# Genie-Kim/PintheMemory

Hardware: AMD Instinct MI355X
Metric: train imgs/sec 768x768 bs=8 R50-DeepLabV3+ +mem (higher is better)
Workload: dtype f32

## Files before the change

include/pinmem_hip.h:

```cpp
#ifndef PINMEM_HIP_H
#define PINMEM_HIP_H
#include <stddef.h>
#include <stdint.h>

#ifdef __cplusplus
extern "C" {
#endif

typedef enum pm_status { PM_OK = 0, PM_EINVAL = -1, PM_EWORKSPACE = -2, PM_ELAUNCH = -3, PM_EUNSUPPORTED = -4 } pm_status;

typedef enum pm_dtype { PM_F32 = 0, PM_BF16 = 1 } pm_dtype;
#define PM_TF_ZERO_PAD64 1

typedef struct pm_tensor {
  void* ptr;
  int32_t n, h, w, c;
  int64_t pitch;
  int32_t dtype;
  int32_t flags;
} pm_tensor;

#define PM_ABI_VERSION 400

typedef struct pm_conv_params {
// ... 6 lines not shown
  int64_t wxf_bytes;
  int32_t wxf_valid;
} pm_conv_params;

typedef struct pm_conv_epilogue {
  int64_t struct_size;
  const float* bias;
  const float* scale;
  const float* shift;
  const float* residual;
  int64_t residual_pitch;
  int32_t relu;
  float* bn_partials;
  int64_t bn_partials_bytes;
} pm_conv_epilogue;

const char* pm_last_error(void);
int pm_version(void);

size_t pm_conv_workspace(const pm_tensor* x, const pm_tensor* y, const pm_conv_params* p, int which );
size_t pm_conv_winograd_v_bytes(const pm_tensor* x, const pm_tensor* y, const pm_conv_params* p);
size_t pm_conv_wxf_bytes(const pm_tensor* x, const pm_tensor* y, const pm_conv_params* p);
size_t pm_conv_wxf_bytes_dgrad(const pm_tensor* dy, const pm_tensor* dx, const pm_conv_params* p);
typedef struct pm_wxf_job {
  const float* w;
  void* wxf;
  int64_t wxf_bytes;
  int32_t cout, kh, kw, cin;
  int32_t dgrad;
  int32_t reserved;
} pm_wxf_job;
int pm_conv_wxf_refresh_bf16(const pm_wxf_job* jobs, int n, void* stream);
int pm_conv_wxf_refresh_f32(const pm_wxf_job* jobs, int n, void* stream);
size_t pm_conv_bn_partials_bytes(const pm_tensor* x, const pm_tensor* y, const pm_conv_params* p);
int pm_conv_fwd(const pm_tensor* x, const float* w_krsc, const pm_tensor* y, const pm_conv_params* p,
                const pm_conv_epilogue* ep, void* ws, size_t ws_bytes, void* stream);
int pm_conv_bwd_data(const pm_tensor* dy, const float* w_krsc, const pm_tensor* dx, const pm_conv_params* p,
                     const pm_tensor* add, void* ws, size_t ws_bytes, void* stream);
int pm_conv_bwd_data_masked(const pm_tensor* dy, const float* w_krsc, const pm_tensor* dx, const pm_conv_params* p,
                            const pm_tensor* add, const uint8_t* add_mask, void* ws, size_t ws_bytes, void* stream);
int pm_conv_bwd_weight(const pm_tensor* x, const pm_tensor* dy, float* dw_krsc, float* dbias, const pm_conv_params* p,
                       void* ws, size_t ws_bytes, void* stream);

typedef struct pm_routing {
  int32_t struct_size;
  int32_t winograd;
// ... 158 lines not shown
```

pinthememory_amd/csrc/conv_igemm.hip:

```cpp
#include <stdlib.h>
#include <algorithm>
#include <type_traits>
#include <vector>

#include "pm_common.h"

#include "conv_igemm_kernel.h"

namespace {

template <int ZL, bool O16 = false>
__global__ __launch_bounds__(256) void splitk_reduce_vec_kernel(const float* __restrict__ ws, int ksplit, long slab, int M, int Nn,
                                                                float* __restrict__ C, long c_pitch, const float* bias,
                                                                const float* scale, const float* shift, const float* residual,
                                                                long res_pitch, int relu, const unsigned char* res_mask) {
  constexpr int GP = 256 / ZL;
  __shared__ float4 red[ZL > 1 ? ZL : 1][GP];
  const int gl = threadIdx.x % GP, zl = threadIdx.x / GP;
  const long groups = (long)M * Nn / 4;
  for (long g0 = (long)blockIdx.x * GP; g0 < groups; g0 += (long)gridDim.x * GP) {
    const long grp = g0 + gl;
    float4 v = make_float4(0.f, 0.f, 0.f, 0.f);
    if (grp < groups)
#pragma unroll 8
// ... 841 lines not shown
  R_S2_PARITY,
  R_WINO_WGRAD,
  R_BF16_WGRAD,
  R_DIRECT_WGRAD,
};
struct ConvRoute {
  RouteKind kind;
  Plan pl;
  WinoPlan wino;
  WinoWgradPlan wino_w;
  Bf16Plan b16;
  pm_conv_params pe;
  S2Native s2n;
  S2ParityPlan s2p;
  Bf16WgradPlan b16w;
  W16Plan w16;
  bool native16;
  size_t ws_bytes;
  size_t class_off, slab_off;
  size_t bias_off;
  size_t x32_off, dy32_off;
  size_t v_keep_bytes;
  size_t wxf_bytes;
  size_t bn_bytes;
};

ConvRoute route_conv(int which, const pm_tensor* x, const pm_tensor* y, const pm_conv_params* p) {
  ConvRoute r{};
  long M, Nn, K;
  gemm_dims(which, x, y, p, M, Nn, K);
  if (which == MODE_FWD) {
    if ((r.wino = wino_plan(x, y->c, p)).use) {
      r.kind = R_WINO, r.ws_bytes = wino_ws(r.wino), r.wxf_bytes = r.wino.u_bytes;
      r.v_keep_bytes = wino_wgrad_pays(x->c, y->c) ? r.wino.v_bytes : 0;
    } else if (p->prec == 2 && (r.b16 = bf16_plan(x, y, p)).use) {
      r.kind = R_BF16, r.pe = *p, r.ws_bytes = bf16_ws(r.b16), r.wxf_bytes = r.b16.wb_bytes;
    } else {
      r.kind = R_DIRECT, r.pl = make_plan(MODE_FWD, M, Nn, K, p->prec != 0), r.ws_bytes = pm_align_up(r.pl.ws_bytes, 256);
    }
    bool bn;
    if (pm_is_bf16(y)) bn = pm_vec8(y) && r.kind == R_BF16 && (r.b16.c16 ? (r.b16.k16.ksplit == 1 && !r.b16.k16.wide) : r.b16.pl.ksplit == 1);
    else if (pm_is_bf16(x) || (y->c & 3) || (y->pitch & 3) || !pm_aligned16(y->ptr)) bn = false;
    else bn = r.kind == R_BF16 ? r.b16.pl.ksplit == 1 : (r.kind == R_DIRECT && p->prec == 0 && r.pl.ksplit == 1 && r.pl.bn >= 64);
    r.bn_bytes = bn ? pm_align_up((size_t)pm_cdiv(pm_pixels(y), 32) * y->c * 2 * sizeof(float), 256) : 0;
  } else if (which == MODE_DGRAD) {
    if (p->stride == 2) {
      if ((r.s2n = s2_native_plan(y, x, p)).ok) {
        r.kind = R_S2_NATIVE, r.ws_bytes = r.s2n.total;
      } else {
        r.kind = R_S2_PARITY, r.s2p = s2_parity_plan(y, x, p);
        r.class_off = 0, r.slab_off = 4 * r.s2p.tmp_bytes;
        r.dy32_off = pm_align_up(r.slab_off + r.s2p.slab_bytes + 256, 256);
        r.ws_bytes = r.dy32_off + upcast_bytes(y);
      }
    } else if (dgrad_bf16_ok(p) && (r.pe = dgrad_as_fwd(p), r.b16 = bf16_plan(y, x, &r.pe)).use) {
      r.kind = R_BF16, r.ws_bytes = bf16_ws(r.b16), r.wxf_bytes = r.b16.wb_bytes;
    } else if ((r.wino = wino_plan(y, x->c, p)).use) {
      r.kind = R_WINO, r.ws_bytes = wino_ws(r.wino);
    } else {
      r.kind = R_DIRECT, r.pl = make_plan(MODE_DGRAD, M, Nn, K, p->prec != 0), r.ws_bytes = pm_align_up(r.pl.ws_bytes, 256);
    }
  } else {
    const bool tier = pm_is_bf16(x) || pm_is_bf16(y);
    r.native16 = pm_is_bf16(x) && pm_is_bf16(y) && y->c >= 32;
    size_t own;
    if (!tier && (r.b16w = bf16_wgrad_plan(x, y, p)).use) {
      r.kind = R_BF16_WGRAD, own = bf16_wgrad_ws(r.b16w);
    } else if (!tier && (r.wino = wino_plan(x, y->c, p, true)).use) {
      r.kind = R_WINO_WGRAD, r.wino_w = wino_wgrad_plan(r.wino, y->c), own = wino_wgrad_ws(r.wino, r.wino_w);
    } else {
      r.kind = R_DIRECT_WGRAD, r.pl = make_plan(MODE_WGRAD, M, Nn, K, p->prec != 0), own = r.pl.ws_bytes;
      if (r.native16) {
        r.pl.kper = (r.pl.kper + 63) / 64 * 64;
        r.pl.ksplit = (int)((K + r.pl.kper - 1) / r.pl.kper);
        r.w16 = wgrad16_plan(x, y, p, M, Nn, K, r.pl.ksplit);
      }
    }
    r.bias_off = pm_align_up(own, 256);
    r.ws_bytes = r.bias_off + pm_align_up((size_t)pm_cdiv(pm_pixels(y), colsum_rows(pm_pixels(y), y->c)) * y->c * sizeof(float), 256) + upcast_bytes(x) + upcast_bytes(y);
    r.x32_off = r.dy32_off = r.ws_bytes;
    if (!r.native16) r.x32_off -= upcast_bytes(x);
// ... 203 lines not shown
  fclose(f);
  return PM_OK;
}

extern "C" size_t pm_conv_workspace(const pm_tensor* x, const pm_tensor* y, const pm_conv_params* p0, int which) {
  const pm_conv_params tp = tier_params(p0, x, y);
  return route_conv(which, x, y, &tp).ws_bytes;
}
extern "C" size_t pm_conv_winograd_v_bytes(const pm_tensor* x, const pm_tensor* y, const pm_conv_params* p0) {
  if (!x || !y || !p0) return 0;
  const pm_conv_params tp = tier_params(p0, x, y);
  return route_conv(MODE_FWD, x, y, &tp).v_keep_bytes;
}
extern "C" size_t pm_conv_wxf_bytes(const pm_tensor* x, const pm_tensor* y, const pm_conv_params* p0) {
  if (!x || !y || !p0) return 0;
  const pm_conv_params tp = tier_params(p0, x, y);
  return route_conv(MODE_FWD, x, y, &tp).wxf_bytes;
}
extern "C" size_t pm_conv_wxf_bytes_dgrad(const pm_tensor* dy, const pm_tensor* dx, const pm_conv_params* p0) {
  if (!dy || !dx || !p0) return 0;
  const pm_conv_params tp = tier_params(p0, dy, dx);
  return route_conv(MODE_DGRAD, dx, dy, &tp).wxf_bytes;
}
extern "C" size_t pm_conv_bn_partials_bytes(const pm_tensor* x, const pm_tensor* y, const pm_conv_params* p0) {
  if (!x || !y || !p0 || check_common(x, y, p0) != PM_OK) return 0;
  const pm_conv_params tp = tier_params(p0, x, y);
  return route_conv(MODE_FWD, x, y, &tp).bn_bytes;
}

extern "C" int pm_conv_wxf_refresh_f32(const pm_wxf_job* jobs, int n, void* stream) {
  PM_REQUIRE(n >= 0 && (jobs || n == 0), PM_EINVAL, "conv_wxf_refresh_f32: bad job table");
  std::vector<const float*> w(n);
  std::vector<float*> U(n);
  std::vector<int> cout(n), cin(n), kp(n), m(n);
  for (int i = 0; i < n; ++i) {
    const pm_wxf_job& q = jobs[i];
    PM_REQUIRE(q.w && q.wxf && q.cout > 0 && q.cin > 0 && q.kh == 3 && q.kw == 3 && q.dgrad == 0, PM_EINVAL,
               "conv_wxf_refresh_f32: job %d: forward transforms of 3x3 filters only", i);
    PM_REQUIRE(pm_aligned16(q.wxf), PM_EINVAL, "conv_wxf_refresh_f32: job %d: buffer must be 16-byte aligned", i);
    const int Kp = (q.cin + BK - 1) / BK * BK;
    const size_t u4 = pm_align_up((size_t)36 * q.cout * Kp * sizeof(float), 256), u2 = pm_align_up((size_t)16 * q.cout * Kp * sizeof(float), 256);
    PM_REQUIRE((size_t)q.wxf_bytes == u4 || (size_t)q.wxf_bytes == u2, PM_EINVAL, "conv_wxf_refresh_f32: job %d: %ld bytes is neither the F(4x4) nor the F(2x2) transform of %d x %d",
               i, (long)q.wxf_bytes, q.cout, q.cin);
    w[i] = q.w, U[i] = (float*)q.wxf, cout[i] = q.cout, cin[i] = q.cin, kp[i] = Kp, m[i] = (size_t)q.wxf_bytes == u4 ? 4 : 2;
  }
  return pm_wino_filter_xf_multi(w.data(), U.data(), cout.data(), cin.data(), kp.data(), m.data(), n, (hipStream_t)stream);
}

extern "C" int pm_conv_fwd(const pm_tensor* x, const float* w, const pm_tensor* y, const pm_conv_params* p0,
                           const pm_conv_epilogue* ep, void* ws, size_t ws_bytes, void* stream) {
  if (int e = check_common(x, y, p0)) return e;
  const pm_conv_params tp = tier_params(p0, x, y);
  const pm_conv_params* p = &tp;
  PM_REQUIRE(!ep || ep->struct_size == (int64_t)sizeof(pm_conv_epilogue), PM_EINVAL,
             "conv_fwd: pm_conv_epilogue.struct_size %ld != %zu -- caller built against another pinmem_hip.h (library ABI %d)", ep ? (long)ep->struct_size : 0l,
             sizeof(pm_conv_epilogue), PM_ABI_VERSION);
  PM_REQUIRE(w && pm_aligned16(w), PM_EINVAL, "conv_fwd: weight null or unaligned");
  pm_conv_epilogue e0 = {(int64_t)sizeof(pm_conv_epilogue), nullptr, nullptr, nullptr, nullptr, 0, 0};
  if (ep) e0 = *ep;
  PM_REQUIRE((e0.scale == nullptr) == (e0.shift == nullptr), PM_EINVAL, "conv_fwd: scale and shift go together");
  const ConvRoute r = route_conv(MODE_FWD, x, y, p);
  if (e0.bn_partials) {
    PM_REQUIRE(!e0.relu && !e0.residual, PM_EINVAL, "conv_fwd: bn_partials are the statistics of the convolution output (no residual / ReLU)");
    PM_REQUIRE(r.bn_bytes != 0 && (size_t)e0.bn_partials_bytes >= r.bn_bytes, PM_EINVAL, "conv_fwd: this call cannot emit bn_partials (ask pm_conv_bn_partials_bytes): %zu needed", r.bn_bytes);
  }
  PM_REQUIRE(ws_bytes >= r.ws_bytes && (ws || r.ws_bytes == 0), PM_EWORKSPACE, "conv_fwd: workspace %zu < %zu", ws_bytes, r.ws_bytes);
  hipStream_t st = (hipStream_t)stream;
  switch (r.kind) {
    case R_WINO: {
// ... 21 lines not shown
  if (int e = check_common(dx, dy, p0)) return e;
  const pm_conv_params tp = tier_params(p0, dy, dx);
  const pm_conv_params* p = &tp;
  PM_REQUIRE(!add || (add->ptr && pm_same_shape(add, dx) && add->dtype == dx->dtype), PM_EINVAL, "conv_bwd_data: `add` must match dx (shape and dtype)");
  PM_REQUIRE(!add || !pm_is_bf16(add) || pm_vec8(add), PM_EINVAL, "conv_bwd_data: bf16 `add` must be 16B aligned with pitch %% 8 == 0");
  PM_REQUIRE(w && pm_aligned16(w), PM_EINVAL, "conv_bwd_data: weight null or unaligned");
  const ConvRoute r = route_conv(MODE_DGRAD, dx, dy, p);
  PM_REQUIRE(ws_bytes >= r.ws_bytes && (ws || r.ws_bytes == 0), PM_EWORKSPACE, "conv_bwd_data: workspace %zu < %zu", ws_bytes, r.ws_bytes);
  if (add_mask) {
    PM_REQUIRE(add && pm_is_f32(add) && pm_is_f32(dy) && pm_vec4(add) && pm_vec4(dx), PM_EINVAL, "conv_bwd_data: a masked `add` is an fp32 tensor with 16-byte rows and c %% 4 == 0");
    PM_REQUIRE(r.kind == R_DIRECT, PM_EUNSUPPORTED,
               "conv_bwd_data: a masked `add` is served by the fp32 implicit-GEMM route only (this call routes to %s)",
               r.kind == R_WINO ? "Winograd" : (r.kind == R_BF16 ? "the bf16 kernels" : "the stride-2 class kernels"));
  }
  hipStream_t st = (hipStream_t)stream;
  const pm_conv_epilogue e1 = {(int64_t)sizeof(pm_conv_epilogue), nullptr, nullptr, nullptr, add ? (const float*)add->ptr : nullptr, add ? add->pitch : 0, 0};
  switch (r.kind) {
    case R_S2_NATIVE: return dgrad_s2_bf16(dy, w, dx, p, add, r.s2n, ws, st);
    case R_S2_PARITY: return dgrad_s2_parity(dy, w, dx, p, add, r, ws, st);
    case R_BF16: {
      char* wext = (p->wxf && (size_t)p->wxf_bytes >= r.b16.wb_bytes) ? (char*)p->wxf : nullptr;
      return conv_bf16(dy, w, dy->c, dx->c, true, dx, &r.pe, r.b16, e1, ws, st, wext, p->wxf_valid != 0);
    }
    case R_WINO: return wino_conv(dy, w, dy->c, dx->c, true, dx, r.wino, e1, ws, st);
    default:
      PM_REQUIRE(pm_is_f32(dy), PM_EUNSUPPORTED, "conv_bwd_data: a bf16 dy needs at least 32 channels and a stride-1 geometry the forward form covers");
      return conv_direct<MODE_DGRAD>(dx, dy, w, p, r.pl, e1, ws, st, add_mask);
  }
}

extern "C" int pm_conv_bwd_weight(const pm_tensor* x0, const pm_tensor* dy0, float* dw, float* dbias, const pm_conv_params* p0, void* ws,
                                  size_t ws_bytes, void* stream) {
  if (int e = check_common(x0, dy0, p0)) return e;
  const pm_conv_params tp = tier_params(p0, x0, dy0);
  const pm_conv_params* p = &tp;
  PM_REQUIRE(dw && pm_aligned16(dw), PM_EINVAL, "conv_bwd_weight: dw null or unaligned");
  const ConvRoute r = route_conv(MODE_WGRAD, x0, dy0, p);
  PM_REQUIRE(ws && ws_bytes >= r.ws_bytes, PM_EWORKSPACE, "conv_bwd_weight: workspace %zu < %zu", ws_bytes, r.ws_bytes);
  hipStream_t st = (hipStream_t)stream;
  const pm_tensor *x = x0, *dy = dy0;
  pm_tensor x32, dy32;
  if (!r.native16 && pm_is_bf16(x0)) {
    if (int e = upcast(x0, (char*)ws + r.x32_off, &x32, st)) return e;
    x = &x32;
  }
  if (pm_is_bf16(dy0) && (!r.native16 || dbias)) {
    if (int e = upcast(dy0, (char*)ws + r.dy32_off, &dy32, st)) return e;
// ... 21 lines not shown
```

pinthememory_amd/csrc/pm_common.h:

```cpp
#pragma once
#include <hip/hip_runtime.h>
#include <algorithm>
#include <atomic>
#include <stdarg.h>
#include <stdint.h>
#include <stdio.h>

#include "../../include/pinmem_hip.h"

void pm_set_error(const char* fmt, ...);

#define PM_REQUIRE(cond, code, ...)      \
  do {                                   \
    if (!(cond)) {                       \
      pm_set_error(__VA_ARGS__);         \
      return (code);                     \
    }                                    \
  } while (0)

static inline int pm_check_launch(const char* what) {
  hipError_t e = hipGetLastError();
  if (e != hipSuccess) {
    pm_set_error("%s: launch failed: %s", what, hipGetErrorString(e));
    return PM_ELAUNCH;
  }
  return PM_OK;
}

static inline bool pm_aligned16(const void* p) { return (reinterpret_cast<uintptr_t>(p) & 15u) == 0; }
static inline int64_t pm_pixels(const pm_tensor* t) { return (int64_t)t->n * t->h * t->w; }
static inline int pm_cdiv(int64_t a, int64_t b) { return (int)((a + b - 1) / b); }
static inline size_t pm_align_up(size_t v, size_t a) { return (v + a - 1) / a * a; }

static inline bool pm_vec_ok(const pm_tensor* t) { return pm_aligned16(t->ptr) && (t->pitch % 4) == 0; }
static inline bool pm_is_f32(const pm_tensor* t) { return t->dtype == PM_F32; }
static inline bool pm_is_bf16(const pm_tensor* t) { return t->dtype == PM_BF16; }
#define PM_REQUIRE_F32(t, who) PM_REQUIRE(!(t) || pm_is_f32(t), PM_EUNSUPPORTED, "%s: fp32 tensors only (got dtype %d)", who, (t)->dtype)
static inline bool pm_vec8(const pm_tensor* t) { return pm_is_bf16(t) && pm_aligned16(t->ptr) && (t->pitch % 8) == 0 && (t->c % 8) == 0; }

struct pm_wino_geom {
  int N, H, W, d, m, TY, TX;
  long tiles;
};
pm_wino_geom pm_wino_make_geom(int n, int h, int w, int d, int m);
int pm_wino_input_xf(const float* x, long pitch, int C, int Kp, const pm_wino_geom& g, float* V, hipStream_t st);
int pm_wino_filter_xf(const float* w, int Cout, int Cin, int Kp, bool dgrad, int m, float* U, hipStream_t st);
int pm_wino_filter_xf_multi(const float* const* w, float* const* U, const int* cout, const int* cin, const int* kp, const int* m, int n, hipStream_t st);
int pm_wino_output_xf(const float* M, int Cout, const pm_wino_geom& g, float* y, long ypitch, const float* bias, const float* scale, const float* shift,
                      const float* residual, long res_pitch, int relu, hipStream_t st);
int pm_wino_fused_f4(const float* V, const float* U, int Cout, int Kp, const pm_wino_geom& g, float* y, long ypitch, const float* bias, const float* scale,
                     const float* shift, const float* residual, long res_pitch, int relu, hipStream_t st);
int pm_wino_dy_xf(const float* dy, long pitch, int Cout, const pm_wino_geom& g, float* Z, hipStream_t st);
int pm_wino_dw_xf(const float* slab, int ks, int Cout, int Cin, int Kp, int m, float* dw, hipStream_t st);

int pm_bf16_cast_rows(const float* x, long pitch, int C, int Cp, long P, void* out, hipStream_t st);
int pm_bf16_cast_weights(const float* w, int Cout, int T, int Cin, int Cp, bool rotate, void* out, hipStream_t st);
struct PmS2Classes {
  int ky0[4], nky[4], kx0[4], nkx[4];
  void* out[4];
};
int pm_bf16_cast_weights_s2(const float* w, int Cout, int kh, int kw, int Cin, int Cp, const PmS2Classes* cl, hipStream_t st);
int pm_bf16_transpose_taps(const float* x, long pitch, int C, int N, int H, int W, int Ho, int Wo, int kh, int kw, int stride, int pad, int dil, void* out,
                           hipStream_t st);

typedef unsigned short pm_bf16;
int pm16_bn_stats(const pm_tensor* x, float* moments, float eps, float* mean, float* invstd, float* running_mean, float* running_var, float momentum, void* ws,
                  size_t ws_bytes, hipStream_t st);
size_t pm16_bn_workspace(const pm_tensor* x);
int pm16_bn_apply_mask(const pm_tensor* x, const float* mean, const float* invstd, const float* gamma, const float* beta, const pm_tensor* res, int relu,
                       const pm_tensor* y, uint8_t* mask, hipStream_t st);
// ... 183 lines not shown
      const long op = (long)(n * Ho + oy) * Wo + ox;
      const unsigned a = *reinterpret_cast<const unsigned*>(arg + op * C + ch), want = (unsigned)(ky * 3 + kx);
      const float4 d = *reinterpret_cast<const float4*>(dy + op * dp + ch);
      g.x += (a & 255u) == want ? d.x : 0.f;
      g.y += ((a >> 8) & 255u) == want ? d.y : 0.f;
      g.z += ((a >> 16) & 255u) == want ? d.z : 0.f;
      g.w += (a >> 24) == want ? d.w : 0.f;
    }
  }
  return g;
}

__device__ __forceinline__ float pm_wave_sum(float v) {
#pragma unroll
  for (int o = 32; o > 0; o >>= 1) v += __shfl_xor(v, o, 64);
  return v;
}
__device__ __forceinline__ float pm_wave_max(float v) {
#pragma unroll
  for (int o = 32; o > 0; o >>= 1) v = fmaxf(v, __shfl_xor(v, o, 64));
  return v;
}

struct pm_lerp {
  int i0, i1;
  float w0, w1;
};
__host__ __device__ __forceinline__ float pm_ac_scale(int in, int out) {
  return out > 1 ? (float)(in - 1) / (float)(out - 1) : 0.f;
}
__device__ __forceinline__ pm_lerp pm_ac_lerp(float scale, int dst, int in) {
  float src = scale * (float)dst;
  int i0 = (int)src;
  if (i0 > in - 1) i0 = in - 1;
  int i1 = i0 + (i0 < in - 1 ? 1 : 0);
  float l1 = src - (float)i0;
  if (l1 < 0.f) l1 = 0.f;
  if (l1 > 1.f) l1 = 1.f;
  pm_lerp r;
  r.i0 = i0;
  r.i1 = i1;
  r.w1 = l1;
  r.w0 = 1.f - l1;
  return r;
}

// ... 23 lines not shown
```

pinthememory_amd/csrc/winograd.hip:

```cpp
#include "pm_common.h"

namespace {

enum { W_BT = 0, W_AT = 1, W_G = 2, W_A = 3, W_GT = 4 };

template <int MT>
__host__ __device__ constexpr float wino_bt(int i, int j) {
  if (MT == 2) {
    constexpr float t[4][4] = {{1, 0, -1, 0}, {0, 1, 1, 0}, {0, -1, 1, 0}, {0, 1, 0, -1}};
    return t[i & 3][j & 3];
  }
  constexpr float t[6][6] = {{4, 0, -5, 0, 1, 0}, {0, -4, -4, 1, 1, 0}, {0, 4, -4, -1, 1, 0}, {0, -2, -1, 2, 1, 0}, {0, 2, -1, -2, 1, 0}, {0, 4, 0, -5, 0, 1}};
  return t[i][j];
}
template <int MT>
__host__ __device__ constexpr float wino_at(int i, int j) {
  if (MT == 2) {
    constexpr float t[2][4] = {{1, 1, 1, 0}, {0, 1, -1, -1}};
    return t[i & 1][j & 3];
  }
  constexpr float t[4][6] = {{1, 1, 1, 1, 1, 0}, {0, 1, -1, 2, -2, 0}, {0, 1, 1, 4, 4, 0}, {0, 1, -1, 8, -8, 1}};
  return t[i][j];
}
template <int MT>
// ... 68 lines not shown

struct TileId {
  int n, ry, rx, ty, tx;
};
__device__ __forceinline__ TileId decode_tile(unsigned tile, const pm_wino_geom& g) {
  TileId t;
  t.tx = (int)(tile % (unsigned)g.TX);
  unsigned q = tile / (unsigned)g.TX;
  t.ty = (int)(q % (unsigned)g.TY);
  q /= (unsigned)g.TY;
  t.rx = (int)(q % (unsigned)g.d);
  q /= (unsigned)g.d;
  t.ry = (int)(q % (unsigned)g.d);
  t.n = (int)(q / (unsigned)g.d);
  return t;
}

template <int MT, int W>
__global__ __launch_bounds__(256) void wino_input_kernel(const float* __restrict__ x, long xp, int C, int Kp, const pm_wino_geom g, float* __restrict__ V) {
  constexpr int A = MT + 2;
  const unsigned kg = Kp / W;
  const unsigned total = (unsigned)g.tiles * kg;
  const long plane = g.tiles * (long)Kp;
  for (unsigned i = blockIdx.x * 256u + threadIdx.x; i < total; i += gridDim.x * 256u) {
    const unsigned tile = i / kg;
    const int c = (int)(i - tile * kg) * W;
    const TileId t = decode_tile(tile, g);
    const bool cok = c < C;
    Vec<W> tt[A][A];
#pragma unroll
    for (int b = 0; b < A; ++b) {
      const int xx = t.rx + g.d * (MT * t.tx + b - 1);
      const bool xok = cok && (unsigned)xx < (unsigned)g.W;
      Vec<W> col[A], o[A];
#pragma unroll
      for (int a = 0; a < A; ++a) {
        const int yy = t.ry + g.d * (MT * t.ty + a - 1);
        col[a] = (xok && (unsigned)yy < (unsigned)g.H) ? vload<W>(x + ((long)(t.n * g.H + yy) * g.W + xx) * xp + c) : vzero<W>();
      }
      mat_apply<MT, W_BT>(col, o);
#pragma unroll
      for (int a = 0; a < A; ++a) tt[a][b] = o[a];
    }
    float* out = V + (long)tile * Kp + c;
#pragma unroll
    for (int a = 0; a < A; ++a) {
      Vec<W> o[A];
// ... 100 lines not shown
#pragma unroll
  for (int a = 0; a < A; ++a) {
    Vec<4> o[A];
    mat_apply<MT, W_G>(gg[a], o);
#pragma unroll
    for (int b = 0; b < A; ++b) {
#pragma unroll
      for (int e = 0; e < 4; ++e)
        if (k + e >= Kr) o[b].v[e] = 0.f;
      vstore<4>(out + (a * A + b) * plane, o[b]);
    }
  }
}
template <int MT, bool DGRAD>
__global__ __launch_bounds__(256) void wino_filter_kernel(const float* __restrict__ w, int Cout, int Cin, int Kp, float* __restrict__ U) {
  __shared__ float sg[9][32][33];
  wino_filter_block<MT, DGRAD>(w, Cout, Cin, Kp, U, blockIdx.x, blockIdx.y, sg);
}

constexpr int WR_BATCH = 48;
struct WinoRefreshJobs {
  const float* w[WR_BATCH];
  float* U[WR_BATCH];
  int cout[WR_BATCH], cin[WR_BATCH], kp[WR_BATCH], m[WR_BATCH];
  int start[WR_BATCH + 1];
  int n;
};
__global__ __launch_bounds__(256) void wino_filter_multi_kernel(const WinoRefreshJobs t) {
  __shared__ float sg[9][32][33];
  int j = 0;
  while (j + 1 < t.n && (int)blockIdx.x >= t.start[j + 1]) ++j;
  const int local = (int)blockIdx.x - t.start[j];
  const int nbx = t.kp[j] / 32;
  const int bx = local % nbx, by = local / nbx;
  if (t.m[j] == 4) wino_filter_block<4, false>(t.w[j], t.cout[j], t.cin[j], t.kp[j], t.U[j], bx, by, sg);
  else wino_filter_block<2, false>(t.w[j], t.cout[j], t.cin[j], t.kp[j], t.U[j], bx, by, sg);
}

template <int MT, int W>
__global__ __launch_bounds__(256) void wino_dy_kernel(const float* __restrict__ dy, long yp, int Cout, const pm_wino_geom g, float* __restrict__ Z) {
  constexpr int A = MT + 2;
  const unsigned cg = Cout / W;
  const unsigned total = (unsigned)g.tiles * cg;
  const long plane = g.tiles * (long)Cout;
  for (unsigned i = blockIdx.x * 256u + threadIdx.x; i < total; i += gridDim.x * 256u) {
    const unsigned tile = i / cg;
    const int c = (int)(i - tile * cg) * W;
    const TileId t = decode_tile(tile, g);
    Vec<W> r[A][MT];
#pragma unroll
    for (int b = 0; b < MT; ++b) {
      const int xx = t.rx + g.d * (MT * t.tx + b);
      Vec<W> col[MT], o[A];
#pragma unroll
      for (int a = 0; a < MT; ++a) {
        const int yy = t.ry + g.d * (MT * t.ty + a);
        col[a] = (yy < g.H && xx < g.W) ? vload<W>(dy + ((long)(t.n * g.H + yy) * g.W + xx) * yp + c) : vzero<W>();
      }
      mat_apply<MT, W_A>(col, o);
// ... 50 lines not shown
}

typedef float f32x16 __attribute__((ext_vector_type(16)));

struct WinoFusedArgs {
  const float* V;
  const float* U;
  float* y;
  long yp;
  int Cout, Kp;
  pm_wino_geom g;
  const float* bias;
  const float* scale;
  const float* shift;
  const float* residual;
  long rp;
  int relu;
  int ncb;
};

constexpr int WF_THREADS = 768, WF_TB = 32, WF_CB = 32, WF_BK = 16, WF_P = 36;
constexpr size_t WF_LDS = (size_t)WF_P * WF_TB * (WF_CB + 1) * sizeof(float);

__device__ __forceinline__ int wf_xcd_remap(int bid, int nwg) {
  const int q = nwg >> 3, r = nwg & 7, xcd = bid & 7, idx = bid >> 3;
  const int base = xcd < r ? xcd * (q + 1) : r * (q + 1) + (xcd - r) * q;
  return base + idx;
}

__global__ __launch_bounds__(WF_THREADS) void wino_fused_f4_kernel(const WinoFusedArgs a) {
  extern __shared__ __align__(16) float4 lds4[];
  const int tid = threadIdx.x, lane = tid & 63, wave = tid >> 6;
  const int lid = wf_xcd_remap(blockIdx.x, gridDim.x);
  const int tb = lid / a.ncb, cb = lid - tb * a.ncb;
  const long tile0 = (long)tb * WF_TB;
  const int co0 = cb * WF_CB;

  const int rem = tid & 255, row = rem >> 2, chunk = rem & 3, pgrp = tid >> 8;
  const bool is_a = row < WF_TB;
  bool valid;
  const float* gp;
  long plane;
  if (is_a) {
    const long tile = tile0 + row;
    valid = tile < a.g.tiles;
    gp = a.V + (valid ? tile : 0) * a.Kp + chunk * 4;
    plane = a.g.tiles * (long)a.Kp;
  } else {
    const int co = co0 + row - WF_TB;
    valid = co < a.Cout;
    gp = a.U + (long)(valid ? co : 0) * a.Kp + chunk * 4;
    plane = (long)a.Cout * a.Kp;
  }
  gp += (long)pgrp * plane;
  const long pstep = 3 * plane;
  const int ldsw = pgrp * 256 + row * 4 + (chunk ^ ((row >> 2) & 3));
// ... 104 lines not shown
  g.tiles = (long)n * d * d * g.TY * g.TX;
  return g;
}

int pm_wino_input_xf(const float* x, long pitch, int C, int Kp, const pm_wino_geom& g, float* V, hipStream_t st) {
  if (g.m == 4) hipLaunchKernelGGL((wino_input_kernel<4, 2>), dim3(nblocks(g.tiles * (Kp / 2))), dim3(256), 0, st, x, pitch, C, Kp, g, V);
  else hipLaunchKernelGGL((wino_input_kernel<2, 4>), dim3(nblocks(g.tiles * (Kp / 4))), dim3(256), 0, st, x, pitch, C, Kp, g, V);
  return pm_check_launch("wino_input");
}

int pm_wino_filter_xf(const float* w, int Cout, int Cin, int Kp, bool dgrad, int m, float* U, hipStream_t st) {
  const int R = dgrad ? Cin : Cout;
  dim3 grid(Kp / 32, pm_cdiv(R, 32));
  if (m == 4) {
    if (dgrad) hipLaunchKernelGGL((wino_filter_kernel<4, true>), grid, dim3(256), 0, st, w, Cout, Cin, Kp, U);
    else hipLaunchKernelGGL((wino_filter_kernel<4, false>), grid, dim3(256), 0, st, w, Cout, Cin, Kp, U);
  } else {
    if (dgrad) hipLaunchKernelGGL((wino_filter_kernel<2, true>), grid, dim3(256), 0, st, w, Cout, Cin, Kp, U);
    else hipLaunchKernelGGL((wino_filter_kernel<2, false>), grid, dim3(256), 0, st, w, Cout, Cin, Kp, U);
  }
  return pm_check_launch("wino_filter");
}

int pm_wino_filter_xf_multi(const float* const* w, float* const* U, const int* cout, const int* cin, const int* kp, const int* m, int n, hipStream_t st) {
  for (int i0 = 0; i0 < n; i0 += WR_BATCH) {
    WinoRefreshJobs t;
    t.n = std::min(WR_BATCH, n - i0);
    long blocks = 0;
    for (int i = 0; i < t.n; ++i) {
      t.w[i] = w[i0 + i], t.U[i] = U[i0 + i], t.cout[i] = cout[i0 + i], t.cin[i] = cin[i0 + i], t.kp[i] = kp[i0 + i], t.m[i] = m[i0 + i];
      t.start[i] = (int)blocks;
      blocks += (long)(kp[i0 + i] / 32) * pm_cdiv(cout[i0 + i], 32);
    }
    t.start[t.n] = (int)blocks;
    if (blocks == 0) continue;
    hipLaunchKernelGGL(wino_filter_multi_kernel, dim3((unsigned)blocks), dim3(256), 0, st, t);
    if (int e = pm_check_launch("wino_filter_multi")) return e;
  }
  return PM_OK;
}

int pm_wino_output_xf(const float* M, int Cout, const pm_wino_geom& g, float* y, long ypitch, const float* bias, const float* scale, const float* shift,
                      const float* residual, long res_pitch, int relu, hipStream_t st) {
  if (g.m == 4)
    hipLaunchKernelGGL((wino_output_kernel<4, 2>), dim3(nblocks(g.tiles * (Cout / 2))), dim3(256), 0, st, M, Cout, g, y, ypitch, bias, scale, shift, residual,
                       res_pitch, relu);
  else
    hipLaunchKernelGGL((wino_output_kernel<2, 4>), dim3(nblocks(g.tiles * (Cout / 4))), dim3(256), 0, st, M, Cout, g, y, ypitch, bias, scale, shift, residual,
                       res_pitch, relu);
  return pm_check_launch("wino_output");
}

int pm_wino_dy_xf(const float* dy, long pitch, int Cout, const pm_wino_geom& g, float* Z, hipStream_t st) {
  if (g.m == 4) hipLaunchKernelGGL((wino_dy_kernel<4, 2>), dim3(nblocks(g.tiles * (Cout / 2))), dim3(256), 0, st, dy, pitch, Cout, g, Z);
  else hipLaunchKernelGGL((wino_dy_kernel<2, 4>), dim3(nblocks(g.tiles * (Cout / 4))), dim3(256), 0, st, dy, pitch, Cout, g, Z);
// ... 24 lines not shown
```

pinthememory_amd/hip/kernels.py:

```python
import ctypes
from ctypes import byref

import os

import torch

from . import lib as L
from .lib import PmConvEpilogue, PmConvParams, check, ptr, stream, tdesc, workspace


def _lib():
    return L.load()


CONV_PREC = 0
ACT_DTYPE = torch.float32


def set_conv_precision(name):
    global CONV_PREC, ACT_DTYPE
    CONV_PREC = {'f32': 0, 'fp32': 0, 'bf16': 2, 'bf16_operands': 2, 'bf16_staged': 1}[name]
    ACT_DTYPE = torch.bfloat16 if name == 'bf16' else torch.float32


# ... 213 lines not shown
        part = torch.empty(npb // 4, dtype=torch.float32, device=x.device) if npb else None
        bn_partials.append(part)
    ep = None
    if bias is not None or scale is not None or residual is not None or relu or part is not None:
        rd = tdesc(residual) if residual is not None else None
        ep = L.conv_epilogue(ptr(bias), ptr(scale), ptr(shift), rd.ptr if rd else None, rd.pitch if rd else 0, 1 if relu else 0, ptr(part),
                            part.numel() * 4 if part is not None else 0)
    check(lib.pm_conv_fwd(byref(xd), w_krsc.data_ptr(), byref(yd), byref(p), byref(ep) if ep else None, ptr(ws), nb, stream()), 'pm_conv_fwd')
    if u_ent is not None:
        ent, version = u_ent
        cur = L.stream_obj()
        ent[3], ent[4] = cur.record_event(), cur.cuda_stream
        ent[1] = version
    return y


def conv_bwd_data(dy, w_krsc, x_shape, stride, pad, dil, add=None, dtype=None, add_mask=None):
    cout, kh, kw, cin = w_krsc.shape
    dx = new(x_shape, dy, dtype=dtype)
    dyd, dxd = tdesc(dy), tdesc(dx)
    p = L.conv_params(kh, kw, stride, pad, dil, CONV_PREC)
    lib = _lib()
    nb, nbu = _sizes(('d', dy.shape, dy.stride(), dy.dtype, dyd.flags, w_krsc.shape, dx.shape, dx.stride(), dx.dtype, stride, pad, dil, CONV_PREC, _GEN[0]),
                     lambda: (lib.pm_conv_workspace(byref(dxd), byref(dyd), byref(p), 1), lib.pm_conv_wxf_bytes_dgrad(byref(dyd), byref(dxd), byref(p))))
    ws = workspace(nb, dy.device) if nb else None
    ad = tdesc(add) if add is not None else None
    u_ent = _wino_u(p, w_krsc, nbu, dgrad=True) if CONV_PREC == 2 else None
    if add_mask is not None:
        check(lib.pm_conv_bwd_data_masked(byref(dyd), w_krsc.data_ptr(), byref(dxd), byref(p), byref(ad), add_mask.data_ptr(), ptr(ws), nb, stream()), 'pm_conv_bwd_data_masked')
    else:
        check(lib.pm_conv_bwd_data(byref(dyd), w_krsc.data_ptr(), byref(dxd), byref(p), byref(ad) if ad else None, ptr(ws), nb, stream()), 'pm_conv_bwd_data')
    if u_ent is not None:
        ent, version = u_ent
        cur = L.stream_obj()
        ent[3], ent[4] = cur.record_event(), cur.cuda_stream
        ent[1] = version
    return dx


def conv_bwd_weight(x, dy, w_shape_krsc, stride, pad, dil, want_bias=False, wino_v=None, on_stream=None):
    cout, kh, kw, cin = w_shape_krsc
    dw = torch.empty(w_shape_krsc, dtype=torch.float32, device=x.device)
    db = torch.empty(cout, dtype=torch.float32, device=x.device) if want_bias else None
    xd, dyd = tdesc(x), tdesc(dy)
    p = L.conv_params(kh, kw, stride, pad, dil, CONV_PREC)
    if wino_v is not None:
        p.wino_v, p.wino_v_bytes = wino_v.data_ptr(), wino_v.numel() * 4
    lib = _lib()
    nb = _sizes(('w', x.shape, x.stride(), x.dtype, dy.shape, dy.stride(), dy.dtype, w_shape_krsc, stride, pad, dil, CONV_PREC, wino_v is not None, _GEN[0]),
                lambda: lib.pm_conv_workspace(byref(xd), byref(dyd), byref(p), 2))
# ... 434 lines not shown
    field = torch.empty(lib.pm_upsample_ce_field_bytes(byref(ld), H, W) // 4, dtype=torch.float32, device=logits.device)
    nb = lib.pm_upsample_wce_workspace(n, H, W)
    ws = workspace(nb, logits.device)
    check(lib.pm_upsample_wce_fwd_field(byref(ld), inv_temp, labels.data_ptr(), H, W, wt.data_ptr(), stride, int(bool(per_image)), out.data_ptr(), field.data_ptr(),
                                        ptr(ws), nb, stream()), 'pm_upsample_wce_fwd_field')
    return out, field


def upsample_wce_bwd_field(logits, label_hw, loss_out, field, gscale, per_image, inv_temp=1.0):
    H, W = label_hw
    dl = new(tuple(logits.shape), logits, pitch_pad=(logits.stride(2) != logits.shape[3]))
    check(_lib().pm_upsample_wce_bwd_field(byref(tdesc(logits)), inv_temp, H, W, int(bool(per_image)), loss_out.data_ptr(), ptr(gscale), field.data_ptr(),
                                           byref(tdesc(dl)), stream()), 'pm_upsample_wce_bwd_field')
    return dl


def refresh_f32_filters():
    if CONV_PREC != 0 or KEEP_WINOGRAD_U is False or not _U_CACHE or not WXF_REFRESH:
        return 0
    import weakref
    dev = torch.cuda.current_device()
    todo = []
    for key, ent in _U_CACHE.items():
        if key[4] != 0 or key[5] or key[3] != dev or not ent[5] or key[1][1] != 3 or key[1][2] != 3:
            continue
        ent[5] = False
        owner = ent[0]() if isinstance(ent[0], weakref.ref) else ent[0]
        if owner is None or owner.data_ptr() != key[0] or ent[1] == owner._version or not ent[2].is_cuda:
            continue
        todo.append((key, ent, owner))
    if not todo:
        return 0
    jobs = (L.PmWxfJob * len(todo))()
    for j, (key, ent, owner) in zip(jobs, todo):
        cout, kh, kw, cin = key[1]
        j.w, j.wxf, j.wxf_bytes, j.cout, j.kh, j.kw, j.cin, j.dgrad = key[0], ent[2].data_ptr(), key[2], cout, kh, kw, cin, 0
        ent[1] = -1
    check(_lib().pm_conv_wxf_refresh_f32(jobs, len(todo), stream()), 'pm_conv_wxf_refresh_f32')
    cur = L.stream_obj()
    raw = cur.cuda_stream
    if raw not in _U_STREAMS:
        _U_STREAMS[raw] = cur
    ev = cur.record_event()
    for key, ent, owner in todo:
        ent[1], ent[3], ent[4] = owner._version, ev, raw
    return len(todo)


def refresh_filters():
    return refresh_bf16_filters() if CONV_PREC == 2 else refresh_f32_filters()


def mem_read_fwd(x, mem, noise=None):
    n, h, w, d = x.shape
    m = mem.shape[0]
    qr = torch.empty((n, h, w, 2 * d), dtype=torch.float32, device=x.device)
    score = torch.empty((n * h * w, m), dtype=torch.float32, device=x.device)
    pmem = torch.empty_like(score)
    check(_lib().pm_mem_read_fwd(byref(tdesc(x)), mem.data_ptr(), m, ptr(noise), byref(tdesc(qr)), score.data_ptr(), pmem.data_ptr(), stream()), 'pm_mem_read_fwd')
# ... 154 lines not shown
```

pinthememory_amd/hip/lib.py:

```python
import ctypes
import os
from ctypes import POINTER, byref, c_char_p, c_float, c_int, c_int32, c_int64, c_size_t, c_void_p

import torch

_HERE = os.path.dirname(os.path.dirname(os.path.abspath(__file__)))
LIB_PATH = os.environ.get('PM_LIB') or os.path.join(_HERE, 'libpinmem_hip.so')


class PmTensor(ctypes.Structure):
    _fields_ = [('ptr', c_void_p), ('n', c_int32), ('h', c_int32), ('w', c_int32), ('c', c_int32), ('pitch', c_int64), ('dtype', c_int32), ('flags', c_int32)]


PM_F32, PM_BF16 = 0, 1
PM_TF_ZERO_PAD64 = 1


class PmSgdEntry(ctypes.Structure):
    _fields_ = [('param', c_void_p), ('grad', c_void_p), ('momentum_buffer', c_void_p), ('numel', c_int64)]


class PmWxfJob(ctypes.Structure):
    _fields_ = [('w', c_void_p), ('wxf', c_void_p), ('wxf_bytes', c_int64), ('cout', c_int32), ('kh', c_int32), ('kw', c_int32), ('cin', c_int32),
                ('dgrad', c_int32), ('reserved', c_int32)]
# ... 19 lines not shown
    return PmConvParams(ctypes.sizeof(PmConvParams), kh, kw, stride, pad, dil, prec)


def conv_epilogue(*fields):
    return PmConvEpilogue(ctypes.sizeof(PmConvEpilogue), *fields)


ABI_VERSION = 400


class PinmemError(RuntimeError):
    pass


_T, _P, _E = POINTER(PmTensor), POINTER(PmConvParams), POINTER(PmConvEpilogue)
_vp, _sz, _i, _f, _i64 = c_void_p, c_size_t, c_int, c_float, c_int64

SIGNATURES = {
    'pm_last_error': (c_char_p, []),
    'pm_version': (c_int, []),
    'pm_conv_winograd_v_bytes': (_sz, [_T, _T, _P]),
    'pm_conv_wxf_bytes': (_sz, [_T, _T, _P]),
    'pm_conv_wxf_bytes_dgrad': (_sz, [_T, _T, _P]),
    'pm_conv_wxf_refresh_bf16': (_i, [_vp, _i, _vp]),
    'pm_conv_wxf_refresh_f32': (_i, [_vp, _i, _vp]),
    'pm_conv_workspace': (_sz, [_T, _T, _P, _i]),
    'pm_conv_fwd': (_i, [_T, _vp, _T, _P, _E, _vp, _sz, _vp]),
    'pm_conv_bwd_data': (_i, [_T, _vp, _T, _P, _T, _vp, _sz, _vp]),
    'pm_conv_bwd_data_masked': (_i, [_T, _vp, _T, _P, _T, _vp, _vp, _sz, _vp]),
    'pm_conv_bwd_weight': (_i, [_T, _T, _vp, _vp, _P, _vp, _sz, _vp]),
    'pm_set_winograd': (_i, [_i]),
    'pm_set_winograd_fused': (_i, [_i]),
    'pm_set_conv16': (_i, [_i]),
    'pm_profile_enable': (_i, [_i]),
    'pm_profile_dump': (_i, [ctypes.c_char_p]),
    'pm_profile_read': (_i, [_i, _i, _i, _i, _i, POINTER(ctypes.c_double), POINTER(ctypes.c_double), POINTER(c_int64), _i]),
    'pm_profile_read_prec': (_i, [_i, _i, _i, _i, _i, _i, POINTER(ctypes.c_double), POINTER(ctypes.c_double), POINTER(c_int64), _i]),
    'pm_profile_read_bytes': (_i, [_i, _i, _i, _i, _i, _i, POINTER(ctypes.c_double)]),
    'pm_bn_workspace': (_sz, [_T]),
    'pm_bn_stats': (_i, [_T, _vp, _vp, _sz, _vp]),
    'pm_bn_merge': (_i, [_vp, _i, _i, _vp, _vp]),
    'pm_bn_merge_finalize': (_i, [_vp, _i, _i, _f, _vp, _vp, _vp, _vp, _f, _vp]),
    'pm_bn_finalize': (_i, [_vp, _i, _f, _vp, _vp, _vp, _vp, _f, _vp]),
    'pm_bn_stats_finalize': (_i, [_T, _f, _vp, _vp, _vp, _vp, _f, _vp, _sz, _vp]),
    'pm_bn_fold': (_i, [_vp, _vp, _vp, _vp, _vp, _i, _f, _vp, _vp, _vp]),
    'pm_bn_fold_multi': (_i, [_vp, _vp, _vp, _i, _i, _i, _f, _vp, _vp]),
# ... 170 lines not shown
```

Baseline: 156.2.

## Cache f32 Winograd dgrad filter transforms and XCD-remap input transform blocks

Extends the cached Winograd filter-transform machinery to the f32 data-gradient path. The transposed 3x3 filter transform is now kept in a per-weight buffer, refreshed in the batched multi-job kernel after weight updates, and passed to wino_conv so the per-call filter transform is skipped when the cache is valid. It also moves the XCD block-remap helper into the common header and applies it to the input-transform kernel to improve L2 locality across chiplets. This adds a persistent buffer per dgrad weight and extra refresh bookkeeping.

After: 156.5, median of 6. No clear change (+0.2%).

```diff
diff --git a/include/pinmem_hip.h b/include/pinmem_hip.h
--- a/include/pinmem_hip.h
+++ b/include/pinmem_hip.h
@@ -52,6 +52,7 @@
 size_t pm_conv_winograd_v_bytes(const pm_tensor* x, const pm_tensor* y, const pm_conv_params* p);
 size_t pm_conv_wxf_bytes(const pm_tensor* x, const pm_tensor* y, const pm_conv_params* p);
 size_t pm_conv_wxf_bytes_dgrad(const pm_tensor* dy, const pm_tensor* dx, const pm_conv_params* p);
+size_t pm_conv_wino_u_bytes_dgrad(const pm_tensor* dy, const pm_tensor* dx, const pm_conv_params* p);
 typedef struct pm_wxf_job {
   const float* w;
   void* wxf;
diff --git a/pinthememory_amd/csrc/conv_igemm.hip b/pinthememory_amd/csrc/conv_igemm.hip
--- a/pinthememory_amd/csrc/conv_igemm.hip
+++ b/pinthememory_amd/csrc/conv_igemm.hip
@@ -887,6 +887,7 @@
   size_t x32_off, dy32_off;
   size_t v_keep_bytes;
   size_t wxf_bytes;
+  size_t wino_u_dgrad_bytes;
   size_t bn_bytes;
 };
 
@@ -921,7 +922,7 @@
     } else if (dgrad_bf16_ok(p) && (r.pe = dgrad_as_fwd(p), r.b16 = bf16_plan(y, x, &r.pe)).use) {
       r.kind = R_BF16, r.ws_bytes = bf16_ws(r.b16), r.wxf_bytes = r.b16.wb_bytes;
     } else if ((r.wino = wino_plan(y, x->c, p)).use) {
-      r.kind = R_WINO, r.ws_bytes = wino_ws(r.wino);
+      r.kind = R_WINO, r.ws_bytes = wino_ws(r.wino), r.wino_u_dgrad_bytes = r.wino.u_bytes;
     } else {
       r.kind = R_DIRECT, r.pl = make_plan(MODE_DGRAD, M, Nn, K, p->prec != 0), r.ws_bytes = pm_align_up(r.pl.ws_bytes, 256);
     }
@@ -1171,6 +1172,11 @@
   const pm_conv_params tp = tier_params(p0, dy, dx);
   return route_conv(MODE_DGRAD, dx, dy, &tp).wxf_bytes;
 }
+extern "C" size_t pm_conv_wino_u_bytes_dgrad(const pm_tensor* dy, const pm_tensor* dx, const pm_conv_params* p0) {
+  if (!dy || !dx || !p0) return 0;
+  const pm_conv_params tp = tier_params(p0, dy, dx);
+  return route_conv(MODE_DGRAD, dx, dy, &tp).wino_u_dgrad_bytes;
+}
 extern "C" size_t pm_conv_bn_partials_bytes(const pm_tensor* x, const pm_tensor* y, const pm_conv_params* p0) {
   if (!x || !y || !p0 || check_common(x, y, p0) != PM_OK) return 0;
   const pm_conv_params tp = tier_params(p0, x, y);
@@ -1181,19 +1187,21 @@
   PM_REQUIRE(n >= 0 && (jobs || n == 0), PM_EINVAL, "conv_wxf_refresh_f32: bad job table");
   std::vector<const float*> w(n);
   std::vector<float*> U(n);
-  std::vector<int> cout(n), cin(n), kp(n), m(n);
+  std::vector<int> cout(n), cin(n), kp(n), m(n), dg(n);
   for (int i = 0; i < n; ++i) {
     const pm_wxf_job& q = jobs[i];
-    PM_REQUIRE(q.w && q.wxf && q.cout > 0 && q.cin > 0 && q.kh == 3 && q.kw == 3 && q.dgrad == 0, PM_EINVAL,
-               "conv_wxf_refresh_f32: job %d: forward transforms of 3x3 filters only", i);
+    PM_REQUIRE(q.w && q.wxf && q.cout > 0 && q.cin > 0 && q.kh == 3 && q.kw == 3 && (q.dgrad == 0 || q.dgrad == 1), PM_EINVAL,
+               "conv_wxf_refresh_f32: job %d: transforms of 3x3 filters only, dgrad 0 or 1", i);
     PM_REQUIRE(pm_aligned16(q.wxf), PM_EINVAL, "conv_wxf_refresh_f32: job %d: buffer must be 16-byte aligned", i);
-    const int Kp = (q.cin + BK - 1) / BK * BK;
-    const size_t u4 = pm_align_up((size_t)36 * q.cout * Kp * sizeof(float), 256), u2 = pm_align_up((size_t)16 * q.cout * Kp * sizeof(float), 256);
-    PM_REQUIRE((size_t)q.wxf_bytes == u4 || (size_t)q.wxf_bytes == u2, PM_EINVAL, "conv_wxf_refresh_f32: job %d: %ld bytes is neither the F(4x4) nor the F(2x2) transform of %d x %d",
-               i, (long)q.wxf_bytes, q.cout, q.cin);
-    w[i] = q.w, U[i] = (float*)q.wxf, cout[i] = q.cout, cin[i] = q.cin, kp[i] = Kp, m[i] = (size_t)q.wxf_bytes == u4 ? 4 : 2;
-  }
-  return pm_wino_filter_xf_multi(w.data(), U.data(), cout.data(), cin.data(), kp.data(), m.data(), n, (hipStream_t)stream);
+    const int rows = q.dgrad ? q.cin : q.cout;
+    const int Kp = ((q.dgrad ? q.cout : q.cin) + BK - 1) / BK * BK;
+    const size_t u4 = pm_align_up((size_t)36 * rows * Kp * sizeof(float), 256), u2 = pm_align_up((size_t)16 * rows * Kp * sizeof(float), 256);
+    PM_REQUIRE((size_t)q.wxf_bytes == u4 || (size_t)q.wxf_bytes == u2, PM_EINVAL,
+               "conv_wxf_refresh_f32: job %d: %ld bytes is neither the F(4x4) nor the F(2x2) %s transform of %d x %d", i, (long)q.wxf_bytes,
+               q.dgrad ? "data-gradient" : "forward", q.cout, q.cin);
+    w[i] = q.w, U[i] = (float*)q.wxf, cout[i] = q.cout, cin[i] = q.cin, kp[i] = Kp, m[i] = (size_t)q.wxf_bytes == u4 ? 4 : 2, dg[i] = q.dgrad;
+  }
+  return pm_wino_filter_xf_multi(w.data(), U.data(), cout.data(), cin.data(), kp.data(), m.data(), dg.data(), n, (hipStream_t)stream);
 }
 
 extern "C" int pm_conv_fwd(const pm_tensor* x, const float* w, const pm_tensor* y, const pm_conv_params* p0,
@@ -1261,7 +1269,10 @@
       char* wext = (p->wxf && (size_t)p->wxf_bytes >= r.b16.wb_bytes) ? (char*)p->wxf : nullptr;
       return conv_bf16(dy, w, dy->c, dx->c, true, dx, &r.pe, r.b16, e1, ws, st, wext, p->wxf_valid != 0);
     }
-    case R_WINO: return wino_conv(dy, w, dy->c, dx->c, true, dx, r.wino, e1, ws, st);
+    case R_WINO: {
+      float* uext = (p->wxf && (size_t)p->wxf_bytes >= r.wino.u_bytes) ? (float*)p->wxf : nullptr;
+      return wino_conv(dy, w, dy->c, dx->c, true, dx, r.wino, e1, ws, st, nullptr, uext, p->wxf_valid != 0);
+    }
     default:
       PM_REQUIRE(pm_is_f32(dy), PM_EUNSUPPORTED, "conv_bwd_data: a bf16 dy needs at least 32 channels and a stride-1 geometry the forward form covers");
       return conv_direct<MODE_DGRAD>(dx, dy, w, p, r.pl, e1, ws, st, add_mask);
diff --git a/pinthememory_amd/csrc/pm_common.h b/pinthememory_amd/csrc/pm_common.h
--- a/pinthememory_amd/csrc/pm_common.h
+++ b/pinthememory_amd/csrc/pm_common.h
@@ -45,7 +45,8 @@
 pm_wino_geom pm_wino_make_geom(int n, int h, int w, int d, int m);
 int pm_wino_input_xf(const float* x, long pitch, int C, int Kp, const pm_wino_geom& g, float* V, hipStream_t st);
 int pm_wino_filter_xf(const float* w, int Cout, int Cin, int Kp, bool dgrad, int m, float* U, hipStream_t st);
-int pm_wino_filter_xf_multi(const float* const* w, float* const* U, const int* cout, const int* cin, const int* kp, const int* m, int n, hipStream_t st);
+int pm_wino_filter_xf_multi(const float* const* w, float* const* U, const int* cout, const int* cin, const int* kp, const int* m, const int* dgrad, int n,
+                            hipStream_t st);
 int pm_wino_output_xf(const float* M, int Cout, const pm_wino_geom& g, float* y, long ypitch, const float* bias, const float* scale, const float* shift,
                       const float* residual, long res_pitch, int relu, hipStream_t st);
 int pm_wino_fused_f4(const float* V, const float* U, int Cout, int Kp, const pm_wino_geom& g, float* y, long ypitch, const float* bias, const float* scale,
@@ -275,6 +276,12 @@
   return v;
 }
 
+__device__ __forceinline__ int pm_xcd_remap(int bid, int nwg) {
+  const int q = nwg >> 3, r = nwg & 7, xcd = bid & 7, idx = bid >> 3;
+  const int base = xcd < r ? xcd * (q + 1) : r * (q + 1) + (xcd - r) * q;
+  return base + idx;
+}
+
 struct pm_lerp {
   int i0, i1;
   float w0, w1;
diff --git a/pinthememory_amd/csrc/winograd.hip b/pinthememory_amd/csrc/winograd.hip
--- a/pinthememory_amd/csrc/winograd.hip
+++ b/pinthememory_amd/csrc/winograd.hip
@@ -114,7 +114,8 @@
   const unsigned kg = Kp / W;
   const unsigned total = (unsigned)g.tiles * kg;
   const long plane = g.tiles * (long)Kp;
-  for (unsigned i = blockIdx.x * 256u + threadIdx.x; i < total; i += gridDim.x * 256u) {
+  const unsigned lid = (unsigned)pm_xcd_remap((int)blockIdx.x, (int)gridDim.x);
+  for (unsigned i = lid * 256u + threadIdx.x; i < total; i += gridDim.x * 256u) {
     const unsigned tile = i / kg;
     const int c = (int)(i - tile * kg) * W;
     const TileId t = decode_tile(tile, g);
@@ -261,7 +262,7 @@
 struct WinoRefreshJobs {
   const float* w[WR_BATCH];
   float* U[WR_BATCH];
-  int cout[WR_BATCH], cin[WR_BATCH], kp[WR_BATCH], m[WR_BATCH];
+  int cout[WR_BATCH], cin[WR_BATCH], kp[WR_BATCH], m[WR_BATCH], dgrad[WR_BATCH];
   int start[WR_BATCH + 1];
   int n;
 };
@@ -272,8 +273,13 @@
   const int local = (int)blockIdx.x - t.start[j];
   const int nbx = t.kp[j] / 32;
   const int bx = local % nbx, by = local / nbx;
-  if (t.m[j] == 4) wino_filter_block<4, false>(t.w[j], t.cout[j], t.cin[j], t.kp[j], t.U[j], bx, by, sg);
-  else wino_filter_block<2, false>(t.w[j], t.cout[j], t.cin[j], t.kp[j], t.U[j], bx, by, sg);
+  if (t.dgrad[j]) {
+    if (t.m[j] == 4) wino_filter_block<4, true>(t.w[j], t.cout[j], t.cin[j], t.kp[j], t.U[j], bx, by, sg);
+    else wino_filter_block<2, true>(t.w[j], t.cout[j], t.cin[j], t.kp[j], t.U[j], bx, by, sg);
+  } else {
+    if (t.m[j] == 4) wino_filter_block<4, false>(t.w[j], t.cout[j], t.cin[j], t.kp[j], t.U[j], bx, by, sg);
+    else wino_filter_block<2, false>(t.w[j], t.cout[j], t.cin[j], t.kp[j], t.U[j], bx, by, sg);
+  }
 }
 
 template <int MT, int W>
@@ -370,16 +376,10 @@
 constexpr int WF_THREADS = 768, WF_TB = 32, WF_CB = 32, WF_BK = 16, WF_P = 36;
 constexpr size_t WF_LDS = (size_t)WF_P * WF_TB * (WF_CB + 1) * sizeof(float);
 
-__device__ __forceinline__ int wf_xcd_remap(int bid, int nwg) {
-  const int q = nwg >> 3, r = nwg & 7, xcd = bid & 7, idx = bid >> 3;
-  const int base = xcd < r ? xcd * (q + 1) : r * (q + 1) + (xcd - r) * q;
-  return base + idx;
-}
-
 __global__ __launch_bounds__(WF_THREADS) void wino_fused_f4_kernel(const WinoFusedArgs a) {
   extern __shared__ __align__(16) float4 lds4[];
   const int tid = threadIdx.x, lane = tid & 63, wave = tid >> 6;
-  const int lid = wf_xcd_remap(blockIdx.x, gridDim.x);
+  const int lid = pm_xcd_remap(blockIdx.x, gridDim.x);
   const int tb = lid / a.ncb, cb = lid - tb * a.ncb;
   const long tile0 = (long)tb * WF_TB;
   const int co0 = cb * WF_CB;
@@ -530,15 +530,17 @@
   return pm_check_launch("wino_filter");
 }
 
-int pm_wino_filter_xf_multi(const float* const* w, float* const* U, const int* cout, const int* cin, const int* kp, const int* m, int n, hipStream_t st) {
+int pm_wino_filter_xf_multi(const float* const* w, float* const* U, const int* cout, const int* cin, const int* kp, const int* m, const int* dgrad, int n,
+                            hipStream_t st) {
   for (int i0 = 0; i0 < n; i0 += WR_BATCH) {
     WinoRefreshJobs t;
     t.n = std::min(WR_BATCH, n - i0);
     long blocks = 0;
     for (int i = 0; i < t.n; ++i) {
       t.w[i] = w[i0 + i], t.U[i] = U[i0 + i], t.cout[i] = cout[i0 + i], t.cin[i] = cin[i0 + i], t.kp[i] = kp[i0 + i], t.m[i] = m[i0 + i];
+      t.dgrad[i] = dgrad[i0 + i] ? 1 : 0;
       t.start[i] = (int)blocks;
-      blocks += (long)(kp[i0 + i] / 32) * pm_cdiv(cout[i0 + i], 32);
+      blocks += (long)(kp[i0 + i] / 32) * pm_cdiv(dgrad[i0 + i] ? cin[i0 + i] : cout[i0 + i], 32);
     }
     t.start[t.n] = (int)blocks;
     if (blocks == 0) continue;
diff --git a/pinthememory_amd/hip/kernels.py b/pinthememory_amd/hip/kernels.py
--- a/pinthememory_amd/hip/kernels.py
+++ b/pinthememory_amd/hip/kernels.py
@@ -259,10 +259,13 @@
     p = L.conv_params(kh, kw, stride, pad, dil, CONV_PREC)
     lib = _lib()
     nb, nbu = _sizes(('d', dy.shape, dy.stride(), dy.dtype, dyd.flags, w_krsc.shape, dx.shape, dx.stride(), dx.dtype, stride, pad, dil, CONV_PREC, _GEN[0]),
-                     lambda: (lib.pm_conv_workspace(byref(dxd), byref(dyd), byref(p), 1), lib.pm_conv_wxf_bytes_dgrad(byref(dyd), byref(dxd), byref(p))))
+                     lambda: (lib.pm_conv_workspace(byref(dxd), byref(dyd), byref(p), 1),
+                              (lib.pm_conv_wxf_bytes_dgrad if CONV_PREC == 2 else lib.pm_conv_wino_u_bytes_dgrad)(byref(dyd), byref(dxd), byref(p))))
     ws = workspace(nb, dy.device) if nb else None
     ad = tdesc(add) if add is not None else None
-    u_ent = _wino_u(p, w_krsc, nbu, dgrad=True) if CONV_PREC == 2 else None
+    u_ent = _wino_u(p, w_krsc, nbu, dgrad=True) if (CONV_PREC == 2 or (CONV_PREC == 0 and kh == 3)) else None
+    if _XFORM_COUNT[1] and CONV_PREC == 0 and p.wxf_valid == 0 and nbu:
+        _XFORM_COUNT[0] += 1
     if add_mask is not None:
         check(lib.pm_conv_bwd_data_masked(byref(dyd), w_krsc.data_ptr(), byref(dxd), byref(p), byref(ad), add_mask.data_ptr(), ptr(ws), nb, stream()), 'pm_conv_bwd_data_masked')
     else:
@@ -743,7 +746,7 @@
     dev = torch.cuda.current_device()
     todo = []
     for key, ent in _U_CACHE.items():
-        if key[4] != 0 or key[5] or key[3] != dev or not ent[5] or key[1][1] != 3 or key[1][2] != 3:
+        if key[4] != 0 or key[3] != dev or not ent[5] or key[1][1] != 3 or key[1][2] != 3:
             continue
         ent[5] = False
         owner = ent[0]() if isinstance(ent[0], weakref.ref) else ent[0]
@@ -755,7 +758,7 @@
     jobs = (L.PmWxfJob * len(todo))()
     for j, (key, ent, owner) in zip(jobs, todo):
         cout, kh, kw, cin = key[1]
-        j.w, j.wxf, j.wxf_bytes, j.cout, j.kh, j.kw, j.cin, j.dgrad = key[0], ent[2].data_ptr(), key[2], cout, kh, kw, cin, 0
+        j.w, j.wxf, j.wxf_bytes, j.cout, j.kh, j.kw, j.cin, j.dgrad = key[0], ent[2].data_ptr(), key[2], cout, kh, kw, cin, 1 if key[5] else 0
         ent[1] = -1
     check(_lib().pm_conv_wxf_refresh_f32(jobs, len(todo), stream()), 'pm_conv_wxf_refresh_f32')
     cur = L.stream_obj()
diff --git a/pinthememory_amd/hip/lib.py b/pinthememory_amd/hip/lib.py
--- a/pinthememory_amd/hip/lib.py
+++ b/pinthememory_amd/hip/lib.py
@@ -65,6 +65,7 @@
     'pm_conv_winograd_v_bytes': (_sz, [_T, _T, _P]),
     'pm_conv_wxf_bytes': (_sz, [_T, _T, _P]),
     'pm_conv_wxf_bytes_dgrad': (_sz, [_T, _T, _P]),
+    'pm_conv_wino_u_bytes_dgrad': (_sz, [_T, _T, _P]),
     'pm_conv_wxf_refresh_bf16': (_i, [_vp, _i, _vp]),
     'pm_conv_wxf_refresh_f32': (_i, [_vp, _i, _vp]),
     'pm_conv_workspace': (_sz, [_T, _T, _P, _i]),
```
